# simonrw/rust-tensorflow-serving2

Hardware: AMD Instinct MI355X
Metric: Predict RPCs/sec + p50 latency, ResNet-50 batch=1/32 at 1/2/4/8 MI355X (higher is better)
Workload: dtype bf16

## Files before the change

### rust_tensorflow_serving2_amd/kernels/halo.hip

```cpp
#include <algorithm>
#include <type_traits>

#include "gemm_epilogue.h"
#include "cgemm.h"

namespace tfsk {

namespace {

using namespace gemm;

__device__ __forceinline__ int halo_key(int lin) { return lin & 7; }

template <int BM, int BN, int WGM, int WGN, int HR, int S_>
struct HG {
  static constexpr int NW = WGM * WGN, NT = 64 * NW;
  static constexpr int WM = BM / WGM, WN = BN / WGN;
  static constexpr int TM = WM / 16, TN = WN / 16;
  static constexpr int HPW = HR / (8 * NW);
  static constexpr int BPW = BN / (8 * NW);
  static constexpr int S = S_;
  static_assert(S == 3 || S == 9, "ring depth must divide the 9 taps (static slots)");
  static constexpr int HALO_B = HR * 128;
  static constexpr int B_B = BN * 128;
  static constexpr int CS_LD = BN + 4;
  static constexpr int LDS_EPI = BM * CS_LD * 4;
  static constexpr int lds(int nbuf) {
    return (nbuf * HALO_B + S * B_B) > LDS_EPI ? (nbuf * HALO_B + S * B_B) : LDS_EPI;
  }
  static_assert(HPW >= 1 && HR % (8 * NW) == 0, "halo DMA split");
  static_assert(BPW >= 1 && BN % (8 * NW) == 0, "B DMA split");
  static_assert(TM >= 1 && TN >= 1 && WM % 16 == 0 && WN % 16 == 0, "wave tile");
  static_assert(HPW + BPW * (S - 2) <= 39, "vmcnt immediate range");
  static_assert(lds(2) <= 160 * 1024, "LDS budget");
};

template <int BM, int BN, int NT, int TM, int TN, int WM, int WN>
__device__ __forceinline__ void halo_epilogue(const IGemmArgs& p, const f32x4 (&acc)[TM][TN], char* smem, int h0,
                                              int w0, int img, int n0, int wm, int wn, int tid, float4 bias0,
                                              float4 bias1) {
  constexpr int CS_LD = BN + 4;
  const int TH = p.TH, TW = p.TW, Ho = p.Ho, Wo = p.Wo;
  const int TI = p.TI > 1 ? p.TI : 1, nimg = p.M / (Ho * Wo);
  const int lane = tid & 63, fr = lane & 15, fq = lane >> 4;
  auto out_row = [&](int row) -> int {
    if (row >= TI * TH * TW) return -1;
    const int ii = row / (TH * TW), r2 = row - ii * (TH * TW);
    const int ph = r2 / TW, pw = r2 - ph * TW;
    const int h = h0 + ph, w = w0 + pw;
    if (h >= Ho || w >= Wo || img + ii >= nimg) return -1;
    return ((img + ii) * Ho + h) * Wo + w;
  };

  if (p.splits <= 1 && p.residual == nullptr && p.out2 == nullptr && !p.out_f32 && p.out != nullptr &&
      p.act != kActGeluErf && !p.epi_f32) {
    constexpr int CB_LD = BN + 8;
    uint16_t* Cb = reinterpret_cast<uint16_t*>(smem);
    const bool use_b = p.bias != nullptr && p.N % 8 == 0;
    const __amdgpu_buffer_rsrc_t rsb =
        __builtin_amdgcn_make_buffer_rsrc(const_cast<float*>(p.bias), 0, use_b ? p.N * 4 : 0, 0x00020000);
    float bj[TN];
#pragma unroll
    for (int j = 0; j < TN; ++j)
      bj[j] = __uint_as_float(
          __builtin_amdgcn_raw_buffer_load_b32(rsb, uint32_t(n0 + wn * WN + j * 16 + fr) * 4u, 0, 0));
    const float alpha = p.alpha;
    dispatch_act<false>(p.act, [&](auto act_tag) __attribute__((always_inline)) {
      constexpr int ACT = decltype(act_tag)::value;
#pragma unroll
      for (int i = 0; i < TM; ++i)
#pragma unroll
        for (int j = 0; j < TN; ++j)
#pragma unroll
          for (int r = 0; r < 4; ++r) {
            const float v = act_fn<ACT>(acc[i][j][r] * alpha + bj[j] + 0.f);
            Cb[(wm * WM + i * 16 + fq * 4 + r) * CB_LD + wn * WN + j * 16 + fr] =
                __builtin_bit_cast(uint16_t, static_cast<__bf16>(v));
          }
    });
    __syncthreads();
    constexpr int CPRB = BN / 8;
#pragma unroll 4
    for (int c = tid; c < BM * CPRB; c += NT) {
      const int row = c / CPRB, ch = c - row * CPRB;
      const int m = out_row(row), n = n0 + ch * 8;
      if (m >= 0 && n < p.N)
        *reinterpret_cast<uint4*>(static_cast<uint16_t*>(p.out) + size_t(m) * p.ldc + n) =
            *reinterpret_cast<const uint4*>(Cb + row * CB_LD + ch * 8);
    }
    return;
  }

  float* Cs = reinterpret_cast<float*>(smem);
#pragma unroll
  for (int i = 0; i < TM; ++i)
#pragma unroll
    for (int j = 0; j < TN; ++j)
#pragma unroll
      for (int r = 0; r < 4; ++r)
        Cs[(wm * WM + i * 16 + fq * 4 + r) * CS_LD + wn * WN + j * 16 + fr] = acc[i][j][r];
  __syncthreads();

  IGemmArgs q = p;
  if (p.splits > 1) {
    splitk_store_slab<BM, BN, NT, CS_LD, kSlabFixup | kSlabRolled>(p, Cs, n0, tid, out_row);
    if (p.counters == nullptr || !splitk_arrive(p, blockIdx.x)) {
      trace_stamp(p, 3);
      return;
    }
    splitk_finish<BM, BN, NT, CS_LD>(q, Cs, n0, tid, out_row, bias0, bias1);
  }
  dispatch_act(q.act, [&](auto act) {
    epilogue_rows<BM, BN, NT, CS_LD, decltype(act)::value, 2>(q, Cs, n0, tid, out_row, bias0, bias1);
  });
}

template <int BM, int BN, int WGM, int WGN, int HR, int S, bool PF>
__global__ __launch_bounds__(64 * WGM * WGN) void halo_conv_kernel(IGemmArgs p) {
  using G = HG<BM, BN, WGM, WGN, HR, S>;
  extern __shared__ __attribute__((aligned(16))) char smem_raw[];
  char* const smem = reinterpret_cast<char*>(smem_raw);
  typedef __attribute__((address_space(3))) void* lds_ptr_t;

  const int TH = p.TH, TW = p.TW, HW2 = TW + 2;
  const int Ho = p.Ho, Wo = p.Wo, H = p.H, W = p.W, C = p.C;
  const int tph = (Ho + TH - 1) / TH, tpw = (Wo + TW - 1) / TW;
  const int nbn = (p.N + BN - 1) / BN;
  const int TI = p.TI > 1 ? p.TI : 1, nimg = p.M / (Ho * Wo);
  const int HB = (TH + 2) * HW2;

  const int wg = xcd_remap(blockIdx.x, gridDim.x);
  const int bn = wg % nbn;
  int r_ = wg / nbn;
  const int tw = r_ % tpw;
  r_ /= tpw;
  const int th = r_ % tph;
  const int img = (r_ / tph) * TI;
  const int h0 = th * TH, w0 = tw * TW, n0 = bn * BN;

  trace_stamp(p, 0);
  const int tid = threadIdx.x, lane = tid & 63;
  const int wid = __builtin_amdgcn_readfirstlane(tid >> 6);
  const int wm = wid / WGN, wn = wid % WGN;
  const int prow = lane >> 3;
  const uint32_t kc = uint32_t(((lane & 7) ^ prow) * 8);

  const __amdgpu_buffer_rsrc_t rsA =
      __builtin_amdgcn_make_buffer_rsrc(const_cast<void*>(p.a), 0, int(p.a_bytes), 0x00020000);
  const __amdgpu_buffer_rsrc_t rsB =
      __builtin_amdgcn_make_buffer_rsrc(const_cast<uint16_t*>(p.b), 0, int(p.b_bytes), 0x00020000);

  const int hrows = TI * HB;
  const float inv_hw2 = 1.f / float(HW2), inv_hb = 1.f / float(HB);
  uint32_t h_off[G::HPW];
#pragma unroll
  for (int j = 0; j < G::HPW; ++j) {
    const int r = (wid * G::HPW + j) * 8 + prow;
    const int ii = TI > 1 ? fdiv(r, HB, inv_hb) : 0;
    const int q = r - ii * HB;
    const int rr = fdiv(q, HW2, inv_hw2);
    const int hh = h0 - p.PT + rr, ww = w0 - p.PL + (q - rr * HW2);
    const bool ok = r < hrows && img + ii < nimg && unsigned(hh) < unsigned(H) && unsigned(ww) < unsigned(W);
    const uint32_t kh = uint32_t(((lane & 7) ^ halo_key(ii * TH * TW + rr * TW + (q - rr * HW2))) * 8);
    h_off[j] = ok ? (uint32_t(((img + ii) * H + hh) * W + ww) * uint32_t(C) + kh) * 2u : kOOB;
  }
  uint32_t b_off[G::BPW];
#pragma unroll
  for (int j = 0; j < G::BPW; ++j) {
    const int n = n0 + (wid * G::BPW + j) * 8 + prow;
    b_off[j] = n < p.N ? (uint32_t(n) * uint32_t(p.ldb) + kc) * 2u : kOOB;
  }

  const int nch = C / KT;
  int c0 = 0, c1 = nch;
  if (p.splits > 1) {
    c0 = blockIdx.y * p.kt_per_split;
    c1 = min(nch, c0 + p.kt_per_split);
  }
  const int nbuf = (c1 - c0) > 1 ? 2 : 1;
  char* const ring = smem + nbuf * G::HALO_B;

  auto issue_halo = [&](int c) {
    char* dst = smem + ((c - c0) & 1) * G::HALO_B;
    const uint32_t soff = uint32_t(c) * (KT * 2);
#pragma unroll
    for (int j = 0; j < G::HPW; ++j) {
      const uint32_t v = h_off[j];
      __builtin_amdgcn_raw_ptr_buffer_load_lds(rsA, (lds_ptr_t)(dst + (wid * G::HPW + j) * 1024), 16, v, soff, 0, 0);
    }
  };
  auto issue_b = [&](int c, int u, int slot) {
    const uint32_t soff = uint32_t(u * C + c * KT) * 2u;
#pragma unroll
    for (int j = 0; j < G::BPW; ++j) {
      const uint32_t v = b_off[j];
      __builtin_amdgcn_raw_ptr_buffer_load_lds(rsB, (lds_ptr_t)(ring + slot * G::B_B + (wid * G::BPW + j) * 1024),
                                               16, v, soff, 0, 0);
    }
  };

  const int fr = lane & 15, fq = lane >> 4;
  int hrow0[G::TM], kpx0[G::TM];
#pragma unroll
  for (int i = 0; i < G::TM; ++i) {
    const int px = wm * G::WM + i * 16 + fr;
    const int ii = px / (TH * TW), p2 = px - ii * (TH * TW);
    const int ph = p2 / TW;
    hrow0[i] = px < TI * TH * TW ? ii * HB + ph * HW2 + (p2 - ph * TW) : 0;
    kpx0[i] = px;
  }
  const uint32_t rb0 = uint32_t(((wn * G::WN + fr) * KT + ((fq ^ (fr & 7)) * 8)) * 2);
  const uint32_t rb1 = uint32_t(((wn * G::WN + fr) * KT + (((4 + fq) ^ (fr & 7)) * 8)) * 2);

  f32x4 acc[G::TM][G::TN];
#pragma unroll
  for (int i = 0; i < G::TM; ++i)
#pragma unroll
    for (int j = 0; j < G::TN; ++j) acc[i][j] = f32x4{0.f, 0.f, 0.f, 0.f};

  struct Frags {
    bf16x8 a[2][G::TM], b[2][G::TN];
  };
  auto load_frags = [&](Frags& f, const char* hb, const char* sb, int tap_off, int tap_key) {
#pragma unroll
    for (int kk = 0; kk < 2; ++kk) {
#pragma unroll
      for (int i = 0; i < G::TM; ++i) {
        const int hr = hrow0[i] + tap_off;
        const uint32_t addr = uint32_t(hr) * 128u + ((uint32_t((kk * 4 + fq) ^ halo_key(kpx0[i] + tap_key))) << 4);
        f.a[kk][i] = *reinterpret_cast<const bf16x8*>(hb + addr);
      }
#pragma unroll
      for (int j = 0; j < G::TN; ++j)
        f.b[kk][j] = *reinterpret_cast<const bf16x8*>(sb + (kk ? rb1 : rb0) + j * 16 * KT * 2);
    }
  };
  auto mma = [&](const Frags& f) {
#pragma unroll
    for (int kk = 0; kk < 2; ++kk)
#pragma unroll
      for (int i = 0; i < G::TM; ++i)
#pragma unroll
        for (int j = 0; j < G::TN; ++j)
          acc[i][j] = __builtin_amdgcn_mfma_f32_16x16x32_bf16(f.a[kk][i], f.b[kk][j], acc[i][j], 0, 0, 0);
  };
  auto compute = [&](const char* hb, const char* sb, int tap_off, int tap_key) {
    Frags f;
    load_frags(f, hb, sb, tap_off, tap_key);
    mma(f);
  };
  Frags prev;

  float4 bias0, bias1;
  prefetch_bias<BM, BN, G::NT>(p, n0, tid, bias0, bias1);

  constexpr int D = G::S - 1;
  const int nck = c1 - c0;
  issue_halo(c0);
#pragma unroll
  for (int j = 0; j < D; ++j)
    if (j < nck * 9) issue_b(c0 + j / 9, j % 9, j % G::S);

  auto chunk = [&](auto last_tag, int c) {
    constexpr bool LAST = decltype(last_tag)::value;
    const char* hb = smem + ((c - c0) & 1) * G::HALO_B;
#pragma unroll
    for (int u = 0; u < 9; ++u) {
      const int nb = LAST ? (D - 1 < 8 - u ? D - 1 : 8 - u) : D - 1;
      const int younger = G::BPW * nb + ((!LAST && u >= 1 && u < D) ? G::HPW : 0);
      switch (younger) {
#define TFSK_W(k) case k: wait_vmcnt<k>(); break;
        TFSK_W(0) TFSK_W(1) TFSK_W(2) TFSK_W(3) TFSK_W(4) TFSK_W(5) TFSK_W(6) TFSK_W(7) TFSK_W(8) TFSK_W(9)
        TFSK_W(10) TFSK_W(11) TFSK_W(12) TFSK_W(13) TFSK_W(14) TFSK_W(15) TFSK_W(16) TFSK_W(17) TFSK_W(18)
        TFSK_W(19) TFSK_W(20) TFSK_W(21) TFSK_W(22) TFSK_W(23) TFSK_W(24) TFSK_W(25) TFSK_W(26) TFSK_W(27)
        TFSK_W(28) TFSK_W(29) TFSK_W(30) TFSK_W(31) TFSK_W(32) TFSK_W(33) TFSK_W(34) TFSK_W(35) TFSK_W(36)
        TFSK_W(37) TFSK_W(38) TFSK_W(39)
#undef TFSK_W
        default: wait_vmcnt<40>(); break;
      }
      lds_barrier();
      if (u == 0 && c == c0) trace_stamp(p, 1);
      if (!LAST && u == 0) issue_halo(c + 1);
      if (!LAST || u + D < 9) issue_b(c + (u + D) / 9, (u + D) % 9, (u + D) % G::S);
      if constexpr (PF) {
        __builtin_amdgcn_sched_barrier(0);
        Frags cur;
        load_frags(cur, hb, ring + (u % G::S) * G::B_B, (u / 3) * HW2 + (u % 3), (u / 3) * TW + (u % 3));
        __builtin_amdgcn_sched_barrier(0);
        if (u > 0 || c > c0) mma(prev);
        __builtin_amdgcn_sched_barrier(0);
        prev = cur;
      } else {
        compute(hb, ring + (u % G::S) * G::B_B, (u / 3) * HW2 + (u % 3), (u / 3) * TW + (u % 3));
      }
    }
  };
  for (int c = c0; c < c1 - 1; ++c) chunk(std::false_type{}, c);
  chunk(std::true_type{}, c1 - 1);
  if constexpr (PF) mma(prev);
  wait_vmcnt<0>();
  __syncthreads();
  trace_stamp(p, 2);

  halo_epilogue<BM, BN, G::NT, G::TM, G::TN, G::WM, G::WN>(p, acc, smem, h0, w0, img, n0, wm, wn, tid, bias0,
                                                              bias1);
  trace_stamp(p, 3);
}

#define TFSK_PERSIST(id, BM, BN, HR) constexpr int kPersistBM = BM, kPersistBN = BN, kPersistHR = HR;
TFSK_HALO_PERSIST_CONFIGS(TFSK_PERSIST)
#undef TFSK_PERSIST
struct HPs {
  static constexpr int BM = kPersistBM, BN = kPersistBN, HR = kPersistHR;
  static constexpr int WGM = 4, WGN = 2, NW = 8, NT = 512;
  static constexpr int WM = BM / WGM, WN = BN / WGN, TM = WM / 16, TN = WN / 16;
  static constexpr int HPW = HR / (8 * NW), BPW = BN / (8 * NW);
  static constexpr int B_B = BN * 128, HALO_B = HR * 128;
  static constexpr int CB_LD = BN + 8;
  static constexpr int STG_B = BM * CB_LD * 2;
  static constexpr int OFF_HALO = 9 * B_B, OFF_STG = OFF_HALO + 2 * HALO_B;
  static constexpr int LDS = OFF_STG + STG_B;
  static constexpr int kStores = BM * (BN / 8) / NT;
  static_assert(HPW * 8 * NW == HR && BPW == 1 && kStores * NT == BM * (BN / 8), "persistent halo split");
  static_assert(LDS <= 160 * 1024, "LDS budget");
};

template <bool TRACE>
__global__ __launch_bounds__(512, 1) void halo_persist_kernel(IGemmArgs p, int ntiles) {
  using G = HPs;
  constexpr int BM = G::BM, BN = G::BN;
  extern __shared__ __attribute__((aligned(16))) char smem_raw[];
  char* const smem = reinterpret_cast<char*>(smem_raw);
  typedef __attribute__((address_space(3))) void* lds_ptr_t;

  const int TH = p.TH, TW = p.TW, HW2 = TW + 2;
  const int Ho = p.Ho, Wo = p.Wo, H = p.H, W = p.W, C = p.C;
  const int tph = (Ho + TH - 1) / TH, tpw = (Wo + TW - 1) / TW;
  const int TI = p.TI > 1 ? p.TI : 1, nimg = p.M / (Ho * Wo);
  const int HB = (TH + 2) * HW2, hrows = TI * HB;
  const int tid = threadIdx.x, lane = tid & 63;
  const int wid = __builtin_amdgcn_readfirstlane(tid >> 6);
  const int wm = wid / G::WGN, wn = wid % G::WGN;
  const int prow = lane >> 3;
  const int fr = lane & 15, fq = lane >> 4;
  if constexpr (TRACE) trace_stamp(p, 0);

  const __amdgpu_buffer_rsrc_t rsA =
      __builtin_amdgcn_make_buffer_rsrc(const_cast<void*>(p.a), 0, int(p.a_bytes), 0x00020000);
  const __amdgpu_buffer_rsrc_t rsB =
      __builtin_amdgcn_make_buffer_rsrc(const_cast<uint16_t*>(p.b), 0, int(p.b_bytes), 0x00020000);
  const __amdgpu_buffer_rsrc_t rsO =
      __builtin_amdgcn_make_buffer_rsrc(p.out, 0, int(long(p.M) * p.ldc * 2), 0x00020000);
  const bool use_b = p.bias != nullptr;
  const __amdgpu_buffer_rsrc_t rsb =
      __builtin_amdgcn_make_buffer_rsrc(const_cast<float*>(p.bias), 0, use_b ? BN * 4 : 0, 0x00020000);

  float bj[G::TN];
#pragma unroll
  for (int j = 0; j < G::TN; ++j)
    bj[j] = __uint_as_float(__builtin_amdgcn_raw_buffer_load_b32(rsb, uint32_t(wn * G::WN + j * 16 + fr) * 4u, 0, 0));
  const float alpha = p.alpha;
  gemm::wait_vmcnt<0>();

  {
    const uint32_t kc = uint32_t(((lane & 7) ^ prow) * 8);
    const int n = wid * 8 + prow;
    const uint32_t boff = (uint32_t(n) * uint32_t(p.ldb) + kc) * 2u;
#pragma unroll
    for (int u = 0; u < 9; ++u)
      __builtin_amdgcn_raw_ptr_buffer_load_lds(rsB, (lds_ptr_t)(smem + u * G::B_B + wid * 1024), 16, boff,
                                               uint32_t(u * C) * 2u, 0, 0);
  }
  const float inv_hw2 = 1.f / float(HW2), inv_hb = 1.f / float(HB);
  auto issue_halo = [&](int t, int b) {
    int r_ = t;
    const int tw = r_ % tpw;
    r_ /= tpw;
    const int th = r_ % tph;
    const int img = (r_ / tph) * TI;
    const int h0 = th * TH, w0 = tw * TW;
    char* dst = smem + G::OFF_HALO + b * G::HALO_B;
#pragma unroll
    for (int j = 0; j < G::HPW; ++j) {
      const int r = (wid * G::HPW + j) * 8 + prow;
      const int ii = TI > 1 ? fdiv(r, HB, inv_hb) : 0;
      const int q = r - ii * HB;
      const int rr = fdiv(q, HW2, inv_hw2);
      const int hh = h0 - p.PT + rr, ww = w0 - p.PL + (q - rr * HW2);
      const bool ok = r < hrows && img + ii < nimg && unsigned(hh) < unsigned(H) && unsigned(ww) < unsigned(W);
      const uint32_t kh = uint32_t(((lane & 7) ^ halo_key(ii * TH * TW + rr * TW + (q - rr * HW2))) * 8);
      const uint32_t off = ok ? (uint32_t(((img + ii) * H + hh) * W + ww) * uint32_t(C) + kh) * 2u : kOOB;
      __builtin_amdgcn_raw_ptr_buffer_load_lds(rsA, (lds_ptr_t)(dst + (wid * G::HPW + j) * 1024), 16, off, 0, 0, 0);
    }
  };

  int hrow0[G::TM], kpx0[G::TM];
#pragma unroll
  for (int i = 0; i < G::TM; ++i) {
    const int px = wm * G::WM + i * 16 + fr;
    const int ii = px / (TH * TW), p2 = px - ii * (TH * TW);
    const int ph = p2 / TW;
    hrow0[i] = px < TI * TH * TW ? ii * HB + ph * HW2 + (p2 - ph * TW) : 0;
    kpx0[i] = px;
  }
  const uint32_t rb0 = uint32_t(((wn * G::WN + fr) * KT + ((fq ^ (fr & 7)) * 8)) * 2);
  const uint32_t rb1 = uint32_t(((wn * G::WN + fr) * KT + (((4 + fq) ^ (fr & 7)) * 8)) * 2);
  constexpr int CPRB = BN / 8;
  uint16_t* const Cb = reinterpret_cast<uint16_t*>(smem + G::OFF_STG);

  int t = blockIdx.x;
  if (t < ntiles) issue_halo(t, 0);
  for (int k = 0; t < ntiles; t += gridDim.x, ++k) {
    const int b = k & 1;
    if (k == 0) gemm::wait_vmcnt<0>();
    else gemm::wait_vmcnt<G::kStores>();
    gemm::lds_barrier();
    if constexpr (TRACE)
      if (k < 2) trace_stamp(p, k == 0 ? 1 : 4);
    const int tn = t + gridDim.x;
    if (tn < ntiles) issue_halo(tn, b ^ 1);
    __builtin_amdgcn_sched_barrier(0);

    f32x4 acc[G::TM][G::TN];
#pragma unroll
    for (int i = 0; i < G::TM; ++i)
#pragma unroll
      for (int j = 0; j < G::TN; ++j) acc[i][j] = f32x4{0.f, 0.f, 0.f, 0.f};
    const char* hb = smem + G::OFF_HALO + b * G::HALO_B;
    struct TapFrags {
      bf16x8 a[2][G::TM], b[2][G::TN];
    };
    auto load_tap = [&](TapFrags& f, int u) __attribute__((always_inline)) {
      const int tap_off = (u / 3) * HW2 + (u % 3), tap_key = (u / 3) * TW + (u % 3);
      const char* sb = smem + u * G::B_B;
#pragma unroll
      for (int kk = 0; kk < 2; ++kk) {
#pragma unroll
        for (int i = 0; i < G::TM; ++i) {
          const int hr = hrow0[i] + tap_off;
          const uint32_t addr = uint32_t(hr) * 128u + ((uint32_t((kk * 4 + fq) ^ halo_key(kpx0[i] + tap_key))) << 4);
          f.a[kk][i] = *reinterpret_cast<const bf16x8*>(hb + addr);
        }
#pragma unroll
        for (int j = 0; j < G::TN; ++j)
          f.b[kk][j] = *reinterpret_cast<const bf16x8*>(sb + (kk ? rb1 : rb0) + j * 16 * KT * 2);
      }
    };
    TapFrags fr2[2];
    load_tap(fr2[0], 0);
#pragma unroll
    for (int u = 0; u < 9; ++u) {
      __builtin_amdgcn_sched_barrier(0);
      if (u < 8) load_tap(fr2[(u + 1) & 1], u + 1);
      __builtin_amdgcn_sched_barrier(0);
      const TapFrags& f = fr2[u & 1];
#pragma unroll
      for (int kk = 0; kk < 2; ++kk)
#pragma unroll
        for (int i = 0; i < G::TM; ++i)
#pragma unroll
          for (int j = 0; j < G::TN; ++j)
            acc[i][j] = __builtin_amdgcn_mfma_f32_16x16x32_bf16(f.a[kk][i], f.b[kk][j], acc[i][j], 0, 0, 0);
    }
    __builtin_amdgcn_sched_barrier(0);
    if constexpr (TRACE)
      if (k < 2) trace_stamp(p, k == 0 ? 2 : 5);

    auto stage = [&](auto act_tag) __attribute__((always_inline)) {
      constexpr int ACT = decltype(act_tag)::value;
#pragma unroll
      for (int i = 0; i < G::TM; ++i)
#pragma unroll
        for (int j = 0; j < G::TN; ++j)
#pragma unroll
          for (int r = 0; r < 4; ++r) {
            const float v = act_fn<ACT>(acc[i][j][r] * alpha + bj[j] + 0.f);
            Cb[(wm * G::WM + i * 16 + fq * 4 + r) * G::CB_LD + wn * G::WN + j * 16 + fr] =
                __builtin_bit_cast(uint16_t, static_cast<__bf16>(v));
          }
    };
    dispatch_act<false>(p.act, stage);
    gemm::lds_barrier();
    {
      int r_ = t;
      const int tw = r_ % tpw;
      r_ /= tpw;
      const int th = r_ % tph;
      const int img = (r_ / tph) * TI;
      const int h0 = th * TH, w0 = tw * TW;
#pragma unroll
      for (int it = 0; it < G::kStores; ++it) {
        const int c = tid + it * G::NT, row = c / CPRB, ch = c - row * CPRB;
        int m = -1;
        if (row < TI * TH * TW) {
          const int ii = row / (TH * TW), r2 = row - ii * (TH * TW);
          const int ph = r2 / TW, pw = r2 - ph * TW;
          const int h = h0 + ph, w = w0 + pw;
          if (h < Ho && w < Wo && img + ii < nimg) m = ((img + ii) * Ho + h) * Wo + w;
        }
        const uint32_t off = m >= 0 ? (uint32_t(m) * uint32_t(p.ldc) + uint32_t(ch * 8)) * 2u : kOOB;
        const u32x4 v = *reinterpret_cast<const u32x4*>(Cb + row * G::CB_LD + ch * 8);
        __builtin_amdgcn_raw_buffer_store_b128(v, rsO, off, 0, 0);
      }
    }
    if constexpr (TRACE)
      if (k == 0) trace_stamp(p, 3);
  }
  gemm::wait_vmcnt<0>();
  if constexpr (TRACE) trace_stamp(p, 6);
}



bool pick_block(int Ho, int Wo, int BM, int HR, int& TH, int& TW) {
  long best_tiles = -1, best_halo = 0;
  for (int tw = 1; tw <= Wo; ++tw) {
    int th = BM / tw < Ho ? BM / tw : Ho;
    while (th >= 1 && (th + 2) * (tw + 2) > HR) --th;
    if (th < 1) continue;
    const int nh = (Ho + th - 1) / th, nw = (Wo + tw - 1) / tw;
    const int bh = (Ho + nh - 1) / nh, bw = (Wo + nw - 1) / nw;
    const long tiles = long(nh) * nw;
    const long halo = long(bh + 2) * (bw + 2);
    if (best_tiles < 0 || tiles < best_tiles || (tiles == best_tiles && halo < best_halo)) {
      best_tiles = tiles;
      best_halo = halo;
      TH = bh;
      TW = bw;
    }
  }
  return best_tiles > 0;
}

int pick_images(const IGemmArgs& a, int BM, int HR) {
  if (a.TH != a.Ho || a.TW != a.Wo) return 1;
  const int nimg = a.M / (a.Ho * a.Wo);
  int ti = std::min(BM / (a.Ho * a.Wo), HR / ((a.Ho + 2) * (a.Wo + 2)));
  ti = std::min(ti, nimg);
  return ti > 1 ? ti : 1;
}

template <int BM, int BN, int WGM, int WGN, int HR, int S, bool PF = false>
hipError_t launch_halo_cfg(const IGemmArgs& a0, hipStream_t s) {
  using G = HG<BM, BN, WGM, WGN, HR, S>;
  IGemmArgs a = a0;
  a.epi_f32 = epi_f32_env();
  if (!pick_block(a.Ho, a.Wo, BM, HR, a.TH, a.TW)) return hipErrorInvalidValue;
  a.TI = pick_images(a, BM, HR);
  const int nch = a.C / KT;
  const int splits = a.splits > 1 ? a.splits : 1;
  if (splits > 1 && a.kt_per_split <= 0) return hipErrorInvalidValue;
  const int per = splits > 1 ? a.kt_per_split : nch;
  const int nimg = a.M / (a.Ho * a.Wo);
  const long tiles = long((nimg + a.TI - 1) / a.TI) * ((a.Ho + a.TH - 1) / a.TH) * ((a.Wo + a.TW - 1) / a.TW) *
                     ((a.N + BN - 1) / BN);
  if (tiles == 0) return hipSuccess;
  if (tiles >= (1L << 31)) return hipErrorInvalidValue;
  const int lds = G::lds(per > 1 ? 2 : 1);
  hipError_t e = ensure_dyn_lds(reinterpret_cast<const void*>(&halo_conv_kernel<BM, BN, WGM, WGN, HR, S, PF>), G::lds(2));
  if (e != hipSuccess) return e;
  hipLaunchKernelGGL((halo_conv_kernel<BM, BN, WGM, WGN, HR, S, PF>), dim3(unsigned(tiles), splits), dim3(G::NT), lds, s,
                     a);
  return hipGetLastError();
}

long persist_geometry(IGemmArgs& a) {
  if (!pick_block(a.Ho, a.Wo, kPersistBM, kPersistHR, a.TH, a.TW)) return -1;
  a.TI = pick_images(a, kPersistBM, kPersistHR);
  const int nimg = a.M / (a.Ho * a.Wo);
  return long((nimg + a.TI - 1) / a.TI) * ((a.Ho + a.TH - 1) / a.TH) * ((a.Wo + a.TW - 1) / a.TW);
}

hipError_t launch_halo_persist(const IGemmArgs& a0, hipStream_t s) {
  using G = HPs;
  IGemmArgs a = a0;
  a.epi_f32 = epi_f32_env();
  if (a.C != KT || a.N != G::BN || !plain_bf16_epilogue(a) || a.counters != nullptr || a.ldc % 8)
    return hipErrorInvalidValue;
  if (long(a.M) * a.ldc * 2 >= 0x7fffffffL) return hipErrorInvalidValue;
  const long tiles = persist_geometry(a);
  if (tiles < 0) return hipErrorInvalidValue;
  if (tiles == 0) return hipSuccess;
  if (tiles >= (1L << 30)) return hipErrorInvalidValue;
  static int cus = 0;
  if (cus == 0) {
    int dev = 0, n = 0;
    if (hipGetDevice(&dev) != hipSuccess || hipDeviceGetAttribute(&n, hipDeviceAttributeMultiprocessorCount, dev) !=
                                                hipSuccess || n <= 0)
      n = 256;
    cus = n;
  }
  const int grid = int(tiles < cus ? tiles : cus);
  if (a.trace != nullptr) {
    hipError_t e = ensure_dyn_lds(reinterpret_cast<const void*>(&halo_persist_kernel<true>), G::LDS);
    if (e != hipSuccess) return e;
    hipLaunchKernelGGL(halo_persist_kernel<true>, dim3(unsigned(grid)), dim3(G::NT), G::LDS, s, a, int(tiles));
    return hipGetLastError();
  }
  hipError_t e = ensure_dyn_lds(reinterpret_cast<const void*>(&halo_persist_kernel<false>), G::LDS);
  if (e != hipSuccess) return e;
  hipLaunchKernelGGL(halo_persist_kernel<false>, dim3(unsigned(grid)), dim3(G::NT), G::LDS, s, a, int(tiles));
  return hipGetLastError();
}

template <bool PF>
hipError_t launch_halo_row(const IGemmArgs& a, int cfg, hipStream_t s) {
  switch (cfg) {
#define TFSK_CASE(id, pf_id, BM, BN, WGM, WGN, HR, S)             \
  case (PF ? (pf_id != 0 ? pf_id : -id) : id):                    \
    if constexpr (!PF || pf_id != 0)                              \
      return launch_halo_cfg<BM, BN, WGM, WGN, HR, S, PF>(a, s);  \
    break;
    TFSK_HALO_CONFIGS(TFSK_CASE)
#undef TFSK_CASE
    default: break;
  }
  return hipErrorInvalidValue;
}

}

long halo_tiles(const IGemmArgs& a0, int cfg) {
  IGemmArgs a = a0;
  a.epi_f32 = epi_f32_env();
  const TileConfig* c = tile_config(cfg);
  if (c == nullptr || (c->family != TileFamily::kHalo && c->family != TileFamily::kHaloPf)) return 0;
  if (!pick_block(a.Ho, a.Wo, c->bm, c->hr, a.TH, a.TW)) return 0;
  const int nimg = a.M / (a.Ho * a.Wo);
  const int ti = pick_images(a, c->bm, c->hr);
  return long((nimg + ti - 1) / ti) * ((a.Ho + a.TH - 1) / a.TH) * ((a.Wo + a.TW - 1) / a.TW) *
         ((a.N + c->bn - 1) / c->bn);
}

bool halo_persist_tiles(int n, int ho, int wo, long& tiles, int& th, int& tw, int& ti) {
  if (n <= 0 || ho <= 0 || wo <= 0 || long(n) * ho * wo >= (1L << 23)) return false;
  IGemmArgs a{};
  a.Ho = ho;
  a.Wo = wo;
  a.M = n * ho * wo;
  tiles = persist_geometry(a);
  th = a.TH;
  tw = a.TW;
  ti = a.TI;
  return tiles > 0;
}

bool halo_supported(const IGemmArgs& a) {
  return a.KH == 3 && a.KW == 3 && a.SH == 1 && a.SW == 1 && a.C % KT == 0 && a.K == 9 * a.C && a.ldb >= a.K &&
         a.ldb % 8 == 0 && a.N % 8 == 0 && a.ldc % 8 == 0 && (!a.residual || a.ldr % 8 == 0) && a.PT >= 0 &&
         a.PT <= 2 && a.PL >= 0 && a.PL <= 2 && a.Ho > 0 && a.Wo > 0 && a.M % (a.Ho * a.Wo) == 0 &&
         a.M < (1 << 23) && int64_t(a.M / (a.Ho * a.Wo)) * a.H * a.W * a.C < (1LL << 30);
}

int halo_config_bm(int cfg) { return halo_cfg_id(cfg) ? tile_config(cfg)->bm : 0; }
int halo_config_bn(int cfg) { return halo_cfg_id(cfg) ? tile_config(cfg)->bn : 0; }

hipError_t halo_launch(const IGemmArgs& a, int cfg, hipStream_t s) {
  if (!halo_cfg_id(cfg) || !halo_supported(a)) return hipErrorInvalidValue;
  switch (tile_config(cfg)->family) {
    case TileFamily::kHaloPersist: return launch_halo_persist(a, s);
    case TileFamily::kHaloPf: return launch_halo_row<true>(a, cfg, s);
    default: return launch_halo_row<false>(a, cfg, s);
  }
}

}
```

Measured before the change: 56260.

## Split halo conv K loop across two wave groups for undersubscribed launches

Adds an intra-block K split to the halo conv kernel. When a launch has no more tiles than CUs, the block doubles its waves into two groups. Each group streams half the input-channel chunks into its own LDS region, and the partial accumulators are exchanged through LDS and summed before a shared epilogue. This targets small-batch layers where too few workgroups leave CUs idle or underused. The cost is doubled LDS per block, an extra exchange and barrier, and launch logic that depends on an env var and the device CU count.

```diff
diff --git a/rust_tensorflow_serving2_amd/kernels/halo.hip b/rust_tensorflow_serving2_amd/kernels/halo.hip
--- a/rust_tensorflow_serving2_amd/kernels/halo.hip
+++ b/rust_tensorflow_serving2_amd/kernels/halo.hip
@@ -12,9 +12,10 @@
 
 __device__ __forceinline__ int halo_key(int lin) { return lin & 7; }
 
-template <int BM, int BN, int WGM, int WGN, int HR, int S_>
+template <int BM, int BN, int WGM, int WGN, int HR, int S_, int KG = 1>
 struct HG {
-  static constexpr int NW = WGM * WGN, NT = 64 * NW;
+  static_assert(KG == 1 || KG == 2, "one or two K groups");
+  static constexpr int NW = WGM * WGN, NT = 64 * NW * KG;
   static constexpr int WM = BM / WGM, WN = BN / WGN;
   static constexpr int TM = WM / 16, TN = WN / 16;
   static constexpr int HPW = HR / (8 * NW);
@@ -25,15 +26,23 @@
   static constexpr int B_B = BN * 128;
   static constexpr int CS_LD = BN + 4;
   static constexpr int LDS_EPI = BM * CS_LD * 4;
+  static constexpr int XCHG_OFF = LDS_EPI;
+  static constexpr int XCHG_B = KG == 2 ? BM * BN * 4 : 0;
+  static constexpr int group(int nbuf) { return nbuf * HALO_B + S * B_B; }
   static constexpr int lds(int nbuf) {
-    return (nbuf * HALO_B + S * B_B) > LDS_EPI ? (nbuf * HALO_B + S * B_B) : LDS_EPI;
+    return KG * group(nbuf) > LDS_EPI + XCHG_B ? KG * group(nbuf) : LDS_EPI + XCHG_B;
   }
   static_assert(HPW >= 1 && HR % (8 * NW) == 0, "halo DMA split");
   static_assert(BPW >= 1 && BN % (8 * NW) == 0, "B DMA split");
   static_assert(TM >= 1 && TN >= 1 && WM % 16 == 0 && WN % 16 == 0, "wave tile");
+  static_assert(KG == 1 || (TM % 2 == 0 && XCHG_OFF % 16 == 0), "K groups: each wave finishes half of its tile rows");
   static_assert(HPW + BPW * (S - 2) <= 39, "vmcnt immediate range");
   static_assert(lds(2) <= 160 * 1024, "LDS budget");
 };
+
+constexpr bool halo_kgroups_fit(int BN, int NW, int HR, int S) {
+  return NW == 4 && BN == 64 && 2 * (2 * HR * 128 + S * BN * 128) <= 160 * 1024;
+}
 
 template <int BM, int BN, int NT, int TM, int TN, int WM, int WN>
 __device__ __forceinline__ void halo_epilogue(const IGemmArgs& p, const f32x4 (&acc)[TM][TN], char* smem, int h0,
@@ -115,9 +124,9 @@
   });
 }
 
-template <int BM, int BN, int WGM, int WGN, int HR, int S, bool PF>
-__global__ __launch_bounds__(64 * WGM * WGN) void halo_conv_kernel(IGemmArgs p) {
-  using G = HG<BM, BN, WGM, WGN, HR, S>;
+template <int BM, int BN, int WGM, int WGN, int HR, int S, bool PF, int KG = 1>
+__global__ __launch_bounds__(64 * WGM * WGN * KG) void halo_conv_kernel(IGemmArgs p) {
+  using G = HG<BM, BN, WGM, WGN, HR, S, KG>;
   extern __shared__ __attribute__((aligned(16))) char smem_raw[];
   char* const smem = reinterpret_cast<char*>(smem_raw);
   typedef __attribute__((address_space(3))) void* lds_ptr_t;
@@ -141,7 +150,9 @@
   trace_stamp(p, 0);
   const int tid = threadIdx.x, lane = tid & 63;
   const int wid = __builtin_amdgcn_readfirstlane(tid >> 6);
-  const int wm = wid / WGN, wn = wid % WGN;
+  const int kg = KG == 2 ? wid / G::NW : 0;
+  const int gw = KG == 2 ? wid - kg * G::NW : wid;
+  const int wm = gw / WGN, wn = gw % WGN;
   const int prow = lane >> 3;
   const uint32_t kc = uint32_t(((lane & 7) ^ prow) * 8);
 
@@ -155,7 +166,7 @@
   uint32_t h_off[G::HPW];
 #pragma unroll
   for (int j = 0; j < G::HPW; ++j) {
-    const int r = (wid * G::HPW + j) * 8 + prow;
+    const int r = (gw * G::HPW + j) * 8 + prow;
     const int ii = TI > 1 ? fdiv(r, HB, inv_hb) : 0;
     const int q = r - ii * HB;
     const int rr = fdiv(q, HW2, inv_hw2);
@@ -167,7 +178,7 @@
   uint32_t b_off[G::BPW];
 #pragma unroll
   for (int j = 0; j < G::BPW; ++j) {
-    const int n = n0 + (wid * G::BPW + j) * 8 + prow;
+    const int n = n0 + (gw * G::BPW + j) * 8 + prow;
     b_off[j] = n < p.N ? (uint32_t(n) * uint32_t(p.ldb) + kc) * 2u : kOOB;
   }
 
@@ -177,16 +188,21 @@
     c0 = blockIdx.y * p.kt_per_split;
     c1 = min(nch, c0 + p.kt_per_split);
   }
+  if constexpr (KG == 2) {
+    c0 = kg * (nch / 2);
+    c1 = c0 + nch / 2;
+  }
   const int nbuf = (c1 - c0) > 1 ? 2 : 1;
-  char* const ring = smem + nbuf * G::HALO_B;
+  char* const gsm = KG == 2 ? smem + kg * G::group(nbuf) : smem;
+  char* const ring = gsm + nbuf * G::HALO_B;
 
   auto issue_halo = [&](int c) {
-    char* dst = smem + ((c - c0) & 1) * G::HALO_B;
+    char* dst = gsm + ((c - c0) & 1) * G::HALO_B;
     const uint32_t soff = uint32_t(c) * (KT * 2);
 #pragma unroll
     for (int j = 0; j < G::HPW; ++j) {
       const uint32_t v = h_off[j];
-      __builtin_amdgcn_raw_ptr_buffer_load_lds(rsA, (lds_ptr_t)(dst + (wid * G::HPW + j) * 1024), 16, v, soff, 0, 0);
+      __builtin_amdgcn_raw_ptr_buffer_load_lds(rsA, (lds_ptr_t)(dst + (gw * G::HPW + j) * 1024), 16, v, soff, 0, 0);
     }
   };
   auto issue_b = [&](int c, int u, int slot) {
@@ -194,7 +210,7 @@
 #pragma unroll
     for (int j = 0; j < G::BPW; ++j) {
       const uint32_t v = b_off[j];
-      __builtin_amdgcn_raw_ptr_buffer_load_lds(rsB, (lds_ptr_t)(ring + slot * G::B_B + (wid * G::BPW + j) * 1024),
+      __builtin_amdgcn_raw_ptr_buffer_load_lds(rsB, (lds_ptr_t)(ring + slot * G::B_B + (gw * G::BPW + j) * 1024),
                                                16, v, soff, 0, 0);
     }
   };
@@ -263,7 +279,7 @@
 
   auto chunk = [&](auto last_tag, int c) {
     constexpr bool LAST = decltype(last_tag)::value;
-    const char* hb = smem + ((c - c0) & 1) * G::HALO_B;
+    const char* hb = gsm + ((c - c0) & 1) * G::HALO_B;
 #pragma unroll
     for (int u = 0; u < 9; ++u) {
       const int nb = LAST ? (D - 1 < 8 - u ? D - 1 : 8 - u) : D - 1;
@@ -302,8 +318,30 @@
   __syncthreads();
   trace_stamp(p, 2);
 
-  halo_epilogue<BM, BN, G::NT, G::TM, G::TN, G::WM, G::WN>(p, acc, smem, h0, w0, img, n0, wm, wn, tid, bias0,
-                                                              bias1);
+  if constexpr (KG == 2) {
+    constexpr int HM = G::TM / 2;
+    f32x4* const xb = reinterpret_cast<f32x4*>(smem + G::XCHG_OFF);
+    const int mine = (wid * HM * G::TN) * 64 + lane;
+    const int theirs = (((1 - kg) * G::NW + gw) * HM * G::TN) * 64 + lane;
+#pragma unroll
+    for (int i = 0; i < HM; ++i)
+#pragma unroll
+      for (int j = 0; j < G::TN; ++j) xb[mine + (i * G::TN + j) * 64] = kg == 0 ? acc[HM + i][j] : acc[i][j];
+    __syncthreads();
+    f32x4 fin[HM][G::TN];
+#pragma unroll
+    for (int i = 0; i < HM; ++i)
+#pragma unroll
+      for (int j = 0; j < G::TN; ++j) {
+        const f32x4 got = xb[theirs + (i * G::TN + j) * 64];
+        fin[i][j] = kg == 0 ? acc[i][j] + got : got + acc[HM + i][j];
+      }
+    halo_epilogue<BM, BN, G::NT, HM, G::TN, G::WM / 2, G::WN>(p, fin, smem, h0, w0, img, n0, wm * 2 + kg, wn, tid,
+                                                               bias0, bias1);
+  } else {
+    halo_epilogue<BM, BN, G::NT, G::TM, G::TN, G::WM, G::WN>(p, acc, smem, h0, w0, img, n0, wm, wn, tid, bias0,
+                                                                bias1);
+  }
   trace_stamp(p, 3);
 }
 
@@ -540,6 +578,23 @@
   return ti > 1 ? ti : 1;
 }
 
+int device_cus() {
+  static int cus = 0;
+  if (cus == 0) {
+    int dev = 0, n = 0;
+    if (hipGetDevice(&dev) != hipSuccess || hipDeviceGetAttribute(&n, hipDeviceAttributeMultiprocessorCount, dev) !=
+                                                hipSuccess || n <= 0)
+      n = 256;
+    cus = n;
+  }
+  return cus;
+}
+
+bool halo_kgroups_env() {
+  const char* e = getenv("TFSERVE_HALO_KGROUPS");
+  return e == nullptr || atoi(e) != 0;
+}
+
 template <int BM, int BN, int WGM, int WGN, int HR, int S, bool PF = false>
 hipError_t launch_halo_cfg(const IGemmArgs& a0, hipStream_t s) {
   using G = HG<BM, BN, WGM, WGN, HR, S>;
@@ -556,6 +611,17 @@
                      ((a.N + BN - 1) / BN);
   if (tiles == 0) return hipSuccess;
   if (tiles >= (1L << 31)) return hipErrorInvalidValue;
+  if constexpr (!PF && halo_kgroups_fit(BN, WGM * WGN, HR, S)) {
+    if (nch >= 2 && nch % 2 == 0 && splits <= 1 && tiles <= device_cus() && halo_kgroups_env()) {
+      using G2 = HG<BM, BN, WGM, WGN, HR, S, 2>;
+      hipError_t e = ensure_dyn_lds(reinterpret_cast<const void*>(&halo_conv_kernel<BM, BN, WGM, WGN, HR, S, PF, 2>),
+                                    G2::lds(2));
+      if (e != hipSuccess) return e;
+      hipLaunchKernelGGL((halo_conv_kernel<BM, BN, WGM, WGN, HR, S, PF, 2>), dim3(unsigned(tiles)), dim3(G2::NT),
+                         G2::lds(nch > 2 ? 2 : 1), s, a);
+      return hipGetLastError();
+    }
+  }
   const int lds = G::lds(per > 1 ? 2 : 1);
   hipError_t e = ensure_dyn_lds(reinterpret_cast<const void*>(&halo_conv_kernel<BM, BN, WGM, WGN, HR, S, PF>), G::lds(2));
   if (e != hipSuccess) return e;
@@ -582,14 +648,7 @@
   if (tiles < 0) return hipErrorInvalidValue;
   if (tiles == 0) return hipSuccess;
   if (tiles >= (1L << 30)) return hipErrorInvalidValue;
-  static int cus = 0;
-  if (cus == 0) {
-    int dev = 0, n = 0;
-    if (hipGetDevice(&dev) != hipSuccess || hipDeviceGetAttribute(&n, hipDeviceAttributeMultiprocessorCount, dev) !=
-                                                hipSuccess || n <= 0)
-      n = 256;
-    cus = n;
-  }
+  const int cus = device_cus();
   const int grid = int(tiles < cus ? tiles : cus);
   if (a.trace != nullptr) {
     hipError_t e = ensure_dyn_lds(reinterpret_cast<const void*>(&halo_persist_kernel<true>), G::LDS);
```

After: 56350 (median of 2 runs). About the same (+0.2%).
